# SMLC-NYSBC/TARGET-VAE

Hardware: AMD Instinct MI355X
Metric: training images/sec (fwd+bwd+Adam), P8 z=2 64x64 bs=256/GPU (higher is better)
Workload: dtype f32 (matrix products: operands as TWO fp16 parts under one power-of-two scale PER ROW of the operand (row / column of the product), 3 fp16 MFMAs per product block -- 2 where one operand is the exact 0 / 1 matrix -- fp32 accumulate: at least as accurate against fp64 as the fp32 matrix pipe (profiles/

## Files before the change

target-vae_amd/csrc/enc_tail_x6_kernels.hpp:

```cpp

#pragma once
#include <hip/hip_runtime.h>
#include "dense_x6_kernels.hpp"

namespace tvae {

constexpr int ET_C = 128;
constexpr int ET_WAVES = 8;
constexpr int ET_THREADS = 64 * ET_WAVES;
constexpr int ET_D = 4;
constexpr int ET_CHUNK = 32;
constexpr int ET_MAXH = 7;

template <int ACT>
__device__ __forceinline__ float et_act(float v, float slope) {
    if (ACT == ACT_LRELU) return v > 0.f ? v : v * slope;
    if (ACT == ACT_TANH) return tanhf(v);
    return v;
}

__device__ __forceinline__ int et_row(int i, int r, int kh) { return 32 * i + 8 * (r >> 2) + (r & 3) + 4 * kh; }

__device__ __forceinline__ void et_split2h(const float (&x)[8], float s, Cell16 (&bf)[3]) {
    const float y[8] = {x[0] * s, x[1] * s, x[2] * s, x[3] * s, x[4] * s, x[5] * s, x[6] * s, x[7] * s};
    split2hx8(y, bf[0], bf[1]);
}
template <int NP>
__device__ __forceinline__ void et_split(const float (&x)[8], Cell16 (&bf)[3]) {
    if (NP == 3) {
        split3x8(x, bf[0], bf[1], bf[2]);
    } else {
#pragma unroll
        for (int q = 0; q < 4; ++q) bf[0].w[q] = bf16_pair(x[2 * q], x[2 * q + 1]);
    }
}

template <int NP>
__device__ __forceinline__ void et_load_a(const uint4* __restrict__ Ws, int t, int i, int kh, int nl, Cell16 (&a)[3]) {
    const uint4* wp = Ws + (2 * t + kh) * ET_C + nl + 32 * i;
#pragma unroll
    for (int p = 0; p < NP; ++p) a[p].u = wp[p * 16 * ET_C];
}
template <int NP>
__device__ __forceinline__ void et_step_mfma(f32x16 (&acc)[4], const uint4* __restrict__ Ws, int t, int kh, int nl,
                                             Cell16 (&a0)[3], Cell16 (&a1)[3], const Cell16 (&bf)[3]) {
    et_load_a<NP>(Ws, t, 1, kh, nl, a1);
    mfma_np<NP>(acc[0], a0, bf);
    __builtin_amdgcn_sched_barrier(0);
    et_load_a<NP>(Ws, t, 2, kh, nl, a0);
    mfma_np<NP>(acc[1], a1, bf);
    __builtin_amdgcn_sched_barrier(0);
    et_load_a<NP>(Ws, t, 3, kh, nl, a1);
    mfma_np<NP>(acc[2], a0, bf);
    __builtin_amdgcn_sched_barrier(0);
    et_load_a<NP>(Ws, (t + 1) & 7, 0, kh, nl, a0);
    mfma_np<NP>(acc[3], a1, bf);
    __builtin_amdgcn_sched_barrier(0);
}

template <int ACT, bool FULL, bool SH = true>
__device__ __forceinline__ void et_fwd_epilogue(f32x16 (&acc)[4], const float* __restrict__ whs, float* __restrict__ H,
                                                long ldh, float* __restrict__ heads, long ldo, const float* __restrict__ bh,
                                                int nh, long n0, long N, int nl, int kh, float slope,
                                                uint4* __restrict__ bitsH) {
    float hs[8];
    unsigned hb[4] = {0u, 0u, 0u, 0u};
#pragma unroll
    for (int o = 0; o < 8; ++o) hs[o] = 0.f;
    const bool in0 = FULL || n0 + nl < N;
    const unsigned loff = (unsigned)(4 * kh * ldh + nl) * 4u;
    const float* wlane = whs + 32 * kh;
    float4 wq[2][2][2];
#pragma unroll
    for (int u = 0; u < 2; ++u) {
        wq[0][u][0] = *reinterpret_cast<const float4*>(wlane + et_row(0, u, 0) * 8);
        wq[0][u][1] = *reinterpret_cast<const float4*>(wlane + et_row(0, u, 0) * 8 + 4);
    }
#pragma unroll
    for (int it = 0; it < 32; ++it) {
        const int cur = it & 1;
        if (it + 1 < 32) {
#pragma unroll
            for (int u = 0; u < 2; ++u) {
                const int rown = et_row((2 * it + 2 + u) >> 4, (2 * it + 2 + u) & 15, 0);
                wq[cur ^ 1][u][0] = *reinterpret_cast<const float4*>(wlane + rown * 8);
                wq[cur ^ 1][u][1] = *reinterpret_cast<const float4*>(wlane + rown * 8 + 4);
            }
        }
#pragma unroll
        for (int u = 0; u < 2; ++u) {
            const int i = (2 * it + u) >> 4, r = (2 * it + u) & 15;
            const float4 w0 = wq[cur][u][0], w1 = wq[cur][u][1];
            char* hrow = reinterpret_cast<char*>(H + (long)et_row(i, r, 0) * ldh + n0);
            const float v = et_act<ACT>(acc[i][r] + w1.w, slope);
            if (ACT == ACT_LRELU) hb[i] |= v > 0.f ? (1u << (8 * (r >> 2) + (r & 3))) : 0u;
            if (SH && in0) __builtin_nontemporal_store(v, reinterpret_cast<float*>(hrow + loff));
            hs[0] = __fmaf_rn(w0.x, v, hs[0]);
            hs[1] = __fmaf_rn(w0.y, v, hs[1]);
            hs[2] = __fmaf_rn(w0.z, v, hs[2]);
            hs[3] = __fmaf_rn(w0.w, v, hs[3]);
            hs[4] = __fmaf_rn(w1.x, v, hs[4]);
            hs[5] = __fmaf_rn(w1.y, v, hs[5]);
            hs[6] = __fmaf_rn(w1.z, v, hs[6]);
        }
#pragma unroll
        for (int o = 0; o < ET_MAXH; ++o) asm volatile("" : "+v"(hs[o]));
        __builtin_amdgcn_sched_barrier(0);
    }
    if (ACT == ACT_LRELU && bitsH) {
#pragma unroll
        for (int i = 0; i < 4; ++i) {
            hb[i] <<= 4 * kh;
            hb[i] |= (unsigned)__shfl_xor((int)hb[i], 32, 64);
        }
        if (kh == 0 && in0) bitsH[n0 + nl] = make_uint4(hb[0], hb[1], hb[2], hb[3]);
    }
    float* hp = heads + n0 + nl;
#pragma unroll
    for (int q = 0; q < 4; ++q) {
        const float ve = hs[2 * q] + __shfl_xor(hs[2 * q], 32, 64);
        const float vo = (2 * q + 1 < ET_MAXH) ? hs[2 * q + 1] + __shfl_xor(hs[2 * q + 1], 32, 64) : 0.f;
        const int o = 2 * q + kh;
        if (o < nh && in0) hp[(long)o * ldo] = (kh ? vo : ve) + bh[o];
    }
}

template <int NP>
static __global__ __launch_bounds__(ET_THREADS, ET_WAVES / 4)
void enc_tail_fwd_x6_kernel(const uint4* __restrict__ W3, int Rpad, const float* __restrict__ X, long ldx,
                            const float* __restrict__ b2, const float* __restrict__ Wh, const float* __restrict__ bh, int nh,
                            float* __restrict__ H, long ldh, float* __restrict__ heads, long ldo, long N, int act,
                            float slope, uint4* __restrict__ bitsH, uint4* __restrict__ bitsA, H3Scale hs) {
    extern __shared__ __attribute__((aligned(16))) uint4 Ws[];
    __shared__ __attribute__((aligned(16))) float whs[ET_C * 8];
    __shared__ float ia_sm[NP == 2 ? ET_C : 1];
    const int tid = threadIdx.x, lane = tid & 63;
    const int wave = __builtin_amdgcn_readfirstlane(tid >> 6);
    const int nl = lane & 31, kh = lane >> 5;
    for (int i = tid; i < NP * 16 * ET_C; i += ET_THREADS) {
        const int row = i & (ET_C - 1), po = i >> 7;
        Ws[i] = W3[(long)po * Rpad + row];
    }
    if (NP == 2 && tid < ET_C) ia_sm[tid] = h3_inv(h3_scale(hs.amax_a[tid]));
    for (int i = tid; i < ET_C * 8; i += ET_THREADS) {
        const int row = i >> 3, o = i & 7;
        whs[i] = o == 7 ? (b2 ? b2[row] : 0.f) : (o < nh ? Wh[o * ET_C + row] : 0.f);
    }
    __syncthreads();

    const long nchunks = (N + ET_CHUNK - 1) / ET_CHUNK;
    const long gw = (long)blockIdx.x * (ET_THREADS / 64) + wave, gstride = (long)gridDim.x * (ET_THREADS / 64);
    if (gw >= nchunks) return;
    const long my = (nchunks - 1 - gw) / gstride + 1;

    const unsigned xlane = (unsigned)(8 * kh * ldx) * 4u;
    auto load_x = [&](long ci, int t, float (&x)[8]) {
        if (ci >= my) ci = my - 1;
        const long n0 = (gw + ci * gstride) * ET_CHUNK;
        const char* p = reinterpret_cast<const char*>(X + (long)(16 * t) * ldx + n0);
        const unsigned off = xlane + 4u * (unsigned)min((long)nl, N - 1 - n0);
#pragma unroll
        for (int j = 0; j < 8; ++j) x[j] = *reinterpret_cast<const float*>(p + (long)j * ldx * 4 + off);
    };

    f32x16 acc[4];
    float x[ET_D][8];
#pragma unroll
    for (int t = 0; t < ET_D; ++t) load_x(0, t, x[t]);
    Cell16 a0[3], a1[3];
    et_load_a<NP>(Ws, 0, 0, kh, nl, a0);
    float sx = 1.f;
    if (NP == 2) sx = h3_scale(h3_wave_max(fmaxf(hs.amax_x[lane], hs.amax_x[64 + lane])));
    const float ix = h3_inv(sx);
    for (long ci = 0; ci < my; ++ci) {
#pragma unroll
        for (int i = 0; i < 4; ++i)
#pragma unroll
            for (int r = 0; r < 16; ++r) acc[i][r] = 0.f;
        unsigned ab[4] = {0u, 0u, 0u, 0u};
#pragma unroll
        for (int t = 0; t < 8; ++t) {
            Cell16 bf[3];
            if (bitsA) {
#pragma unroll
                for (int j = 0; j < 8; ++j) ab[t >> 1] |= x[t % ET_D][j] > 0.f ? (1u << (16 * (t & 1) + j)) : 0u;
            }
            if (NP == 2) et_split2h(x[t % ET_D], sx, bf);
            else et_split<NP>(x[t % ET_D], bf);
            load_x(ci + (t + ET_D) / 8, (t + ET_D) % 8, x[t % ET_D]);
            et_step_mfma<NP>(acc, Ws, t, kh, nl, a0, a1, bf);
        }
        if (NP == 2) {
#pragma unroll
            for (int i = 0; i < 4; ++i)
#pragma unroll
                for (int r = 0; r < 16; ++r) acc[i][r] = (acc[i][r] * ia_sm[et_row(i, r, kh)]) * ix;
        }
        const long n0 = (gw + ci * gstride) * ET_CHUNK;
        if (bitsA) {
#pragma unroll
            for (int i = 0; i < 4; ++i) {
                ab[i] <<= 8 * kh;
                ab[i] |= (unsigned)__shfl_xor((int)ab[i], 32, 64);
            }
            if (kh == 0 && n0 + nl < N) bitsA[n0 + nl] = make_uint4(ab[0], ab[1], ab[2], ab[3]);
        }
#define TVAE_ET_EPI(A_)                                                                                    \
    do {                                                                                                  \
        if (!H) et_fwd_epilogue<A_, false, false>(acc, whs, H, ldh, heads, ldo, bh, nh, n0, N, nl, kh, slope, bitsH); \
        else if (n0 + ET_CHUNK <= N) et_fwd_epilogue<A_, true>(acc, whs, H, ldh, heads, ldo, bh, nh, n0, N, nl, kh, slope, bitsH); \
        else et_fwd_epilogue<A_, false>(acc, whs, H, ldh, heads, ldo, bh, nh, n0, N, nl, kh, slope, bitsH); \
    } while (0)
        if (act == ACT_LRELU) TVAE_ET_EPI(ACT_LRELU);
        else if (act == ACT_TANH) TVAE_ET_EPI(ACT_TANH);
        else TVAE_ET_EPI(ACT_NONE);
#undef TVAE_ET_EPI
    }
}

__device__ __forceinline__ float et_mask(unsigned w, int bit, float slope) { return (w >> bit) & 1u ? 1.f : slope; }

template <int NP>
static __global__ __launch_bounds__(ET_THREADS, ET_WAVES / 4)
void enc_tail_dgrad_x6_kernel(const uint4* __restrict__ W3p, int Rpad, const uint4* __restrict__ Wh3, int Rpadh,
                              const float* __restrict__ dheads, long ldd, int nh, const uint4* __restrict__ bitsH,
                              const uint4* __restrict__ bitsA, float* __restrict__ dA1, long lda, long N, float slope,
                              const float* __restrict__ amax_a) {
    constexpr int NP1 = NP == 2 ? 3 : NP;
    extern __shared__ __attribute__((aligned(16))) uint4 Ws[];
    uint4* Whs = Ws + NP * 16 * ET_C;
    const int tid = threadIdx.x, lane = tid & 63;
    const int wave = __builtin_amdgcn_readfirstlane(tid >> 6);
    const int nl = lane & 31, kh = lane >> 5;
    for (int i = tid; i < NP * 16 * ET_C; i += ET_THREADS) Ws[i] = W3p[(long)(i >> 7) * Rpad + (i & (ET_C - 1))];
    for (int i = tid; i < NP1 * 2 * ET_C; i += ET_THREADS) Whs[i] = Wh3[(long)(i >> 7) * Rpadh + (i & (ET_C - 1))];
    __shared__ float ia_sm[NP == 2 ? ET_C : 1];
    if (NP == 2 && tid < ET_C) ia_sm[tid] = h3_inv(h3_scale(amax_a[tid]));
    __syncthreads();

    const long nchunks = (N + ET_CHUNK - 1) / ET_CHUNK;
    const long gw = (long)blockIdx.x * (ET_THREADS / 64) + wave, gstride = (long)gridDim.x * (ET_THREADS / 64);
    if (gw >= nchunks) return;
    const long my = (nchunks - 1 - gw) / gstride + 1;

    float dh[8];
    uint4 wHn, wAn;
    auto load_in = [&](long ci) {
        if (ci >= my) ci = my - 1;
        const long n = min((gw + ci * gstride) * ET_CHUNK + nl, N - 1);
#pragma unroll
        for (int o = 0; o < ET_MAXH; ++o) dh[o] = o < nh ? dheads[(long)o * ldd + n] : 0.f;
        dh[7] = 0.f;
        wHn = bitsH[n];
        wAn = bitsA[n];
    };
    Cell16 dcell[3];
    unsigned wHs[4], wAs[4], wAsn[4];
    auto consume = [&]() {
        et_split<NP1>(dh, dcell);
        if (kh) {
#pragma unroll
            for (int p = 0; p < NP1; ++p) dcell[p].u = make_uint4(0u, 0u, 0u, 0u);
        }
        wHs[0] = wHn.x >> (4 * kh); wHs[1] = wHn.y >> (4 * kh); wHs[2] = wHn.z >> (4 * kh); wHs[3] = wHn.w >> (4 * kh);
        wAsn[0] = wAn.x >> (4 * kh); wAsn[1] = wAn.y >> (4 * kh); wAsn[2] = wAn.z >> (4 * kh); wAsn[3] = wAn.w >> (4 * kh);
    };
    f32x16 acc[4], G[4];
    float gs = 1.f;
    auto g_phase = [&]() {
#pragma unroll
        for (int i = 0; i < 4; ++i) {
            Cell16 wc[3];
#pragma unroll
            for (int p = 0; p < NP1; ++p) wc[p].u = Whs[(p * 2 + kh) * ET_C + 32 * i + nl];
#pragma unroll
            for (int r = 0; r < 16; ++r) G[i][r] = 0.f;
            mfma_np<NP1>(G[i], wc, dcell);
        }
        if (NP == 2) {
            float mx = 0.f;
#pragma unroll
            for (int i = 0; i < 4; ++i)
#pragma unroll
                for (int r = 0; r < 16; ++r) mx = fmaxf(mx, fabsf(G[i][r]));
            gs = h3_scale(h3_wave_max(mx));
        }
    };
    load_in(0);
    consume();
    load_in(1);
    g_phase();
    Cell16 a0[3], a1[3];
    et_load_a<NP>(Ws, 0, 0, kh, nl, a0);
    const unsigned loff = (unsigned)(4 * kh * lda + nl) * 4u;
    for (long ci = 0; ci < my; ++ci) {
#pragma unroll
        for (int i = 0; i < 4; ++i) {
            wAs[i] = wAsn[i];
#pragma unroll
            for (int r = 0; r < 16; ++r) acc[i][r] = 0.f;
        }
        const float gs_c = gs, inv_c = NP == 2 ? h3_inv(gs) : 1.f;
#pragma unroll
        for (int u = 0; u < 8; ++u) {
            float xv[8];
#pragma unroll
            for (int j = 0; j < 8; ++j) {
                const int r = 8 * (u & 1) + j;
                xv[j] = G[u >> 1][r] * et_mask(wHs[u >> 1], 8 * (r >> 2) + (r & 3), slope);
            }
            Cell16 bf[3];
            if (NP == 2) et_split2h(xv, gs_c, bf);
            else et_split<NP>(xv, bf);
            et_step_mfma<NP>(acc, Ws, u, kh, nl, a0, a1, bf);
        }
        consume();
        load_in(ci + 2);
        g_phase();
        const long n0 = (gw + ci * gstride) * ET_CHUNK;
        const bool in0 = n0 + nl < N;
#pragma unroll
        for (int i = 0; i < 4; ++i)
#pragma unroll
            for (int r = 0; r < 16; ++r) {
                char* drow = reinterpret_cast<char*>(dA1 + (long)et_row(i, r, 0) * lda + n0);
                const float v = (NP == 2 ? (acc[i][r] * ia_sm[et_row(i, r, kh)]) * inv_c : acc[i][r]) * et_mask(wAs[i], 8 * (r >> 2) + (r & 3), slope);
                if (in0) __builtin_nontemporal_store(v, reinterpret_cast<float*>(drow + loff));
            }
    }
}


constexpr int EW_NC = 32;
constexpr int EW_RAW = ET_C * EW_NC * 4;
constexpr int EW_AUX = 1024;
constexpr int EW_BITS = 1024;
constexpr int EW_STAGE = EW_RAW + EW_AUX + EW_BITS;
constexpr int EW_CELLS = 3 * 4 * ET_C * 16;
constexpr int EW_LDS = 2 * EW_STAGE + 4 * EW_CELLS;

#define TVAE_EW_DMA_X4(dst, src) \
    asm volatile("s_mov_b32 m0, %0\n\ts_nop 0\n\tglobal_load_lds_dwordx4 %1, off" ::"s"(dst), "v"(src) : "memory", "m0")

template <int NP>
static __global__ __launch_bounds__(ET_THREADS, 2) void enc_tail_wgrad_x6_kernel(
    const float* __restrict__ A1, long lda, const float* __restrict__ dheads, long ldd, int nh,
    const uint4* __restrict__ bitsH, const float* __restrict__ Wh, float* __restrict__ slabs, long N, float slope,
    const float* __restrict__ amax_a1, const float* __restrict__ amax_dh) {
    extern __shared__ __attribute__((aligned(16))) unsigned char ew_sm[];
    __shared__ float red_[NP == 2 ? 2 * ET_C : 1];
    const int tid = threadIdx.x, lane = tid & 63;
    const int wave = __builtin_amdgcn_readfirstlane(tid >> 6);
    const unsigned lds0 = (unsigned)(size_t)(__attribute__((address_space(3))) void*)ew_sm;
    uint4* cellsD = reinterpret_cast<uint4*>(ew_sm + 2 * EW_STAGE);
    uint4* cellsA = reinterpret_cast<uint4*>(ew_sm + 2 * EW_STAGE + EW_CELLS);
    const long nchunks = N / EW_NC;
    const long per = (nchunks + gridDim.x - 1) / gridDim.x;
    const long c_beg = (long)blockIdx.x * per;
    const long c_end = c_beg + per < nchunks ? c_beg + per : nchunks;
    const int row = tid & 127, oct = tid >> 7;
    float wh[ET_MAXH];
#pragma unroll
    for (int h = 0; h < ET_MAXH; ++h) wh[h] = h < nh ? Wh[(long)h * ET_C + row] : 0.f;
    float sA = 1.f, sD = 1.f;
    float* is_sm = reinterpret_cast<float*>(red_);
    if (NP == 2) {
        float rs = 0.f;
#pragma unroll
        for (int h = 0; h < ET_MAXH; ++h) rs += fabsf(wh[h]);
        sA = h3_scale(amax_a1[row]);
        sD = h3_scale(amax_dh[0] * rs);
        if (oct == 0) {
            is_sm[row] = h3_inv(sD);
            is_sm[ET_C + row] = h3_inv(sA);
        }
        __syncthreads();
    }
    const float* a_src[2];
#pragma unroll
    for (int q = 0; q < 2; ++q) {
        const int r_ = 8 * (2 * wave + q) + (lane >> 3);
        a_src[q] = A1 + (long)r_ * lda + 4 * ((lane & 7) ^ ((r_ >> 1) & 7));
    }
    const int hrow = (lane >> 3) < nh ? (lane >> 3) : 0;
    const float* h_src = dheads + (long)hrow * ldd + 4 * (lane & 7);
    auto dma_chunk = [&](long ch, int stage) {
        const long n0 = ch * EW_NC;
        const unsigned st = lds0 + (unsigned)(stage * EW_STAGE);
#pragma unroll
        for (int q = 0; q < 2; ++q) {
            const float* src = a_src[q] + n0;
            const unsigned dst = st + (unsigned)((2 * wave + q) * 1024);
            TVAE_EW_DMA_X4(dst, src);
        }
        if (wave == 1) {
            const uint4* src = bitsH + n0 + (lane & 31);
            const unsigned dst = st + (unsigned)(EW_RAW + EW_AUX);
            TVAE_EW_DMA_X4(dst, src);
        } else {
            const float* src = h_src + n0;
            const unsigned dst = st + (unsigned)EW_RAW;
            TVAE_EW_DMA_X4(dst, src);
        }
    };
    f32x16 acc[2];
#pragma unroll
    for (int j = 0; j < 2; ++j)
#pragma unroll
        for (int r = 0; r < 16; ++r) acc[j][r] = 0.f;
    const int ti = wave >> 1, tj = 2 * (wave & 1), kh = lane >> 5, li = lane & 31;
    auto build = [&](int stage, int cb) {
        const unsigned char* sb = ew_sm + stage * EW_STAGE;
        uint4* cD = cellsD + cb * (2 * EW_CELLS / 16);
        uint4* cA = cellsA + cb * (2 * EW_CELLS / 16);
        {
            const float4* rp = reinterpret_cast<const float4*>(sb + row * (EW_NC * 4));
            const int sw = (row >> 1) & 7;
            const float4 v0 = rp[(2 * oct) ^ sw], v1 = rp[(2 * oct + 1) ^ sw];
            const float x[8] = {v0.x, v0.y, v0.z, v0.w, v1.x, v1.y, v1.z, v1.w};
            Cell16 c3[3];
            if (NP == 2) et_split2h(x, sA, c3);
            else et_split<NP>(x, c3);
#pragma unroll
            for (int p = 0; p < NP; ++p) cA[(p * 4 + oct) * ET_C + row] = c3[p].u;
        }
        {
            const float* hs = reinterpret_cast<const float*>(sb + EW_RAW) + oct * 8;
            const unsigned* bw = reinterpret_cast<const unsigned*>(sb + EW_RAW + EW_AUX) + (row >> 5);
            float g[8] = {0.f, 0.f, 0.f, 0.f, 0.f, 0.f, 0.f, 0.f};
#pragma unroll
            for (int h = 0; h < ET_MAXH; ++h) {
                const float4 d0 = *reinterpret_cast<const float4*>(hs + h * EW_NC);
                const float4 d1 = *reinterpret_cast<const float4*>(hs + h * EW_NC + 4);
                g[0] = __fmaf_rn(wh[h], d0.x, g[0]); g[1] = __fmaf_rn(wh[h], d0.y, g[1]);
                g[2] = __fmaf_rn(wh[h], d0.z, g[2]); g[3] = __fmaf_rn(wh[h], d0.w, g[3]);
                g[4] = __fmaf_rn(wh[h], d1.x, g[4]); g[5] = __fmaf_rn(wh[h], d1.y, g[5]);
                g[6] = __fmaf_rn(wh[h], d1.z, g[6]); g[7] = __fmaf_rn(wh[h], d1.w, g[7]);
            }
#pragma unroll
            for (int j = 0; j < 8; ++j) {
                const unsigned w = bw[(oct * 8 + j) * 4];
                g[j] *= ((w >> (row & 31)) & 1u) ? 1.f : slope;
            }
            Cell16 c3[3];
            if (NP == 2) et_split2h(g, sD, c3);
            else et_split<NP>(g, c3);
#pragma unroll
            for (int p = 0; p < NP; ++p) cD[(p * 4 + oct) * ET_C + row] = c3[p].u;
        }
    };
    if (c_beg < c_end) {
        dma_chunk(c_beg, 0);
        asm volatile("s_waitcnt vmcnt(0)" ::: "memory");
        __syncthreads();
        dma_chunk(c_beg + 1 < c_end ? c_beg + 1 : c_beg, 1);
        build(0, 0);
    }
    for (long ch = c_beg; ch < c_end; ++ch) {
        const int cb = (int)((ch - c_beg) & 1);
        asm volatile("s_waitcnt vmcnt(0)" ::: "memory");
        __syncthreads();
        dma_chunk(ch + 2 < c_end ? ch + 2 : c_end - 1, cb);
        const uint4* cD = cellsD + cb * (2 * EW_CELLS / 16);
        const uint4* cA = cellsA + cb * (2 * EW_CELLS / 16);
#pragma unroll
        for (int ks = 0; ks < 2; ++ks) {
            Cell16 af[3], bf[2][3];
#pragma unroll
            for (int p = 0; p < NP; ++p) {
                af[p].u = cD[(p * 4 + 2 * ks + kh) * ET_C + 32 * ti + li];
                bf[0][p].u = cA[(p * 4 + 2 * ks + kh) * ET_C + 32 * tj + li];
                bf[1][p].u = cA[(p * 4 + 2 * ks + kh) * ET_C + 32 * (tj + 1) + li];
            }
            mfma_np<NP>(acc[0], af, bf[0]);
            mfma_np<NP>(acc[1], af, bf[1]);
        }
        build(cb ^ 1, cb ^ 1);
#pragma unroll
        for (int g_ = 0; g_ < 4 * NP; ++g_) {
            __builtin_amdgcn_sched_group_barrier(0x008, 1, 0);
            __builtin_amdgcn_sched_group_barrier(0x100, 3, 0);
            __builtin_amdgcn_sched_group_barrier(0x002, 14, 0);
            __builtin_amdgcn_sched_group_barrier(0x200, 1, 0);
        }
    }
    asm volatile("s_waitcnt vmcnt(0)" ::: "memory");
    float* slab = slabs + (long)blockIdx.x * ET_C * ET_C;
#pragma unroll
    for (int j = 0; j < 2; ++j)
#pragma unroll
        for (int r = 0; r < 16; ++r)
            slab[(long)et_row(ti, r, kh) * ET_C + 32 * (tj + j) + li] =
                NP == 2 ? (acc[j][r] * is_sm[et_row(ti, r, kh)]) * is_sm[ET_C + 32 * (tj + j) + li] : acc[j][r];
}

}
```

Measured before the change: 27590.

## Use 64x64 wave blocks with K-split in encoder-tail wgrad, DPP head reduction

```diff
diff --git a/target-vae_amd/csrc/enc_tail_x6_kernels.hpp b/target-vae_amd/csrc/enc_tail_x6_kernels.hpp
--- a/target-vae_amd/csrc/enc_tail_x6_kernels.hpp
+++ b/target-vae_amd/csrc/enc_tail_x6_kernels.hpp
@@ -338,6 +338,13 @@
 constexpr int EW_STAGE = EW_RAW + EW_AUX + EW_BITS;
 constexpr int EW_CELLS = 3 * 4 * ET_C * 16;
 constexpr int EW_LDS = 2 * EW_STAGE + 4 * EW_CELLS;
+#ifdef TVAE_EW_BLOCK32
+constexpr bool EW_B64 = false;
+#else
+constexpr bool EW_B64 = true;
+#endif
+constexpr int EW_PART = 4 * 64 * 64 * 4;
+static_assert(EW_PART <= 4 * EW_CELLS, "the partial sums reuse the cell sets after the loop");
 
 #define TVAE_EW_DMA_X4(dst, src) \
     asm volatile("s_mov_b32 m0, %0\n\ts_nop 0\n\tglobal_load_lds_dwordx4 %1, off" ::"s"(dst), "v"(src) : "memory", "m0")
@@ -403,12 +410,14 @@
             TVAE_EW_DMA_X4(dst, src);
         }
     };
-    f32x16 acc[2];
-#pragma unroll
-    for (int j = 0; j < 2; ++j)
+    constexpr int NACC = EW_B64 ? 4 : 2;
+    f32x16 acc[NACC];
+#pragma unroll
+    for (int j = 0; j < NACC; ++j)
 #pragma unroll
         for (int r = 0; r < 16; ++r) acc[j][r] = 0.f;
     const int ti = wave >> 1, tj = 2 * (wave & 1), kh = lane >> 5, li = lane & 31;
+    const int half = wave >> 2, bi = (wave >> 1) & 1, bj = wave & 1;
     auto build = [&](int stage, int cb) {
         const unsigned char* sb = ew_sm + stage * EW_STAGE;
         uint4* cD = cellsD + cb * (2 * EW_CELLS / 16);
@@ -428,6 +437,23 @@
             const float* hs = reinterpret_cast<const float*>(sb + EW_RAW) + oct * 8;
             const unsigned* bw = reinterpret_cast<const unsigned*>(sb + EW_RAW + EW_AUX) + (row >> 5);
             float g[8] = {0.f, 0.f, 0.f, 0.f, 0.f, 0.f, 0.f, 0.f};
+#ifndef TVAE_EW_BLOCK32
+            const int jq = (lane & 15) < 14 ? (lane & 15) : 13;
+            const float4 dq = *reinterpret_cast<const float4*>(hs + (jq >> 1) * EW_NC + 4 * (jq & 1));
+#define TVAE_EW_DPP(N_) " row_newbcast:" #N_ " row_mask:0xf bank_mask:0xf bound_ctrl:1\n\t"
+#define TVAE_EW_ROW(H_, LO_, HI_)                                                                                         \
+    asm("s_nop 1\n\t"                                                                                                     \
+        "v_fmac_f32_dpp %0, %8, %12" TVAE_EW_DPP(LO_) "v_fmac_f32_dpp %1, %9, %12" TVAE_EW_DPP(LO_)                          \
+        "v_fmac_f32_dpp %2, %10, %12" TVAE_EW_DPP(LO_) "v_fmac_f32_dpp %3, %11, %12" TVAE_EW_DPP(LO_)                        \
+        "v_fmac_f32_dpp %4, %8, %12" TVAE_EW_DPP(HI_) "v_fmac_f32_dpp %5, %9, %12" TVAE_EW_DPP(HI_)                          \
+        "v_fmac_f32_dpp %6, %10, %12" TVAE_EW_DPP(HI_) "v_fmac_f32_dpp %7, %11, %12" TVAE_EW_DPP(HI_)                        \
+        : "+v"(g[0]), "+v"(g[1]), "+v"(g[2]), "+v"(g[3]), "+v"(g[4]), "+v"(g[5]), "+v"(g[6]), "+v"(g[7])                  \
+        : "v"(dq.x), "v"(dq.y), "v"(dq.z), "v"(dq.w), "v"(wh[H_]))
+            TVAE_EW_ROW(0, 0, 1); TVAE_EW_ROW(1, 2, 3); TVAE_EW_ROW(2, 4, 5); TVAE_EW_ROW(3, 6, 7);
+            TVAE_EW_ROW(4, 8, 9); TVAE_EW_ROW(5, 10, 11); TVAE_EW_ROW(6, 12, 13);
+#undef TVAE_EW_ROW
+#undef TVAE_EW_DPP
+#else
 #pragma unroll
             for (int h = 0; h < ET_MAXH; ++h) {
                 const float4 d0 = *reinterpret_cast<const float4*>(hs + h * EW_NC);
@@ -437,6 +463,7 @@
                 g[4] = __fmaf_rn(wh[h], d1.x, g[4]); g[5] = __fmaf_rn(wh[h], d1.y, g[5]);
                 g[6] = __fmaf_rn(wh[h], d1.z, g[6]); g[7] = __fmaf_rn(wh[h], d1.w, g[7]);
             }
+#endif
 #pragma unroll
             for (int j = 0; j < 8; ++j) {
                 const unsigned w = bw[(oct * 8 + j) * 4];
@@ -463,19 +490,37 @@
         dma_chunk(ch + 2 < c_end ? ch + 2 : c_end - 1, cb);
         const uint4* cD = cellsD + cb * (2 * EW_CELLS / 16);
         const uint4* cA = cellsA + cb * (2 * EW_CELLS / 16);
-#pragma unroll
-        for (int ks = 0; ks < 2; ++ks) {
-            Cell16 af[3], bf[2][3];
-#pragma unroll
-            for (int p = 0; p < NP; ++p) {
-                af[p].u = cD[(p * 4 + 2 * ks + kh) * ET_C + 32 * ti + li];
-                bf[0][p].u = cA[(p * 4 + 2 * ks + kh) * ET_C + 32 * tj + li];
-                bf[1][p].u = cA[(p * 4 + 2 * ks + kh) * ET_C + 32 * (tj + 1) + li];
-            }
-            mfma_np<NP>(acc[0], af, bf[0]);
-            mfma_np<NP>(acc[1], af, bf[1]);
+        if (EW_B64) {
+            Cell16 af[2][3], bf[2][3];
+#pragma unroll
+            for (int p = 0; p < NP; ++p)
+#pragma unroll
+                for (int i = 0; i < 2; ++i) {
+                    af[i][p].u = cD[(p * 4 + 2 * half + kh) * ET_C + 64 * bi + 32 * i + li];
+                    bf[i][p].u = cA[(p * 4 + 2 * half + kh) * ET_C + 64 * bj + 32 * i + li];
+                }
+#pragma unroll
+            for (int pa = 0; pa < NP; ++pa)
+#pragma unroll
+                for (int pb = 0; pb < NP - pa; ++pb)
+#pragma unroll
+                    for (int t = 0; t < 4; ++t) mfma_part<NP>(acc[t], af[t >> 1][pa], bf[t & 1][pb]);
+        } else {
+#pragma unroll
+            for (int ks = 0; ks < 2; ++ks) {
+                Cell16 af[3], bf[2][3];
+#pragma unroll
+                for (int p = 0; p < NP; ++p) {
+                    af[p].u = cD[(p * 4 + 2 * ks + kh) * ET_C + 32 * ti + li];
+                    bf[0][p].u = cA[(p * 4 + 2 * ks + kh) * ET_C + 32 * tj + li];
+                    bf[1][p].u = cA[(p * 4 + 2 * ks + kh) * ET_C + 32 * (tj + 1) + li];
+                }
+                mfma_np<NP>(acc[0], af, bf[0]);
+                mfma_np<NP>(acc[1], af, bf[1]);
+            }
         }
         build(cb ^ 1, cb ^ 1);
+#ifdef TVAE_EW_BLOCK32
 #pragma unroll
         for (int g_ = 0; g_ < 4 * NP; ++g_) {
             __builtin_amdgcn_sched_group_barrier(0x008, 1, 0);
@@ -483,15 +528,38 @@
             __builtin_amdgcn_sched_group_barrier(0x002, 14, 0);
             __builtin_amdgcn_sched_group_barrier(0x200, 1, 0);
         }
+#endif
     }
     asm volatile("s_waitcnt vmcnt(0)" ::: "memory");
     float* slab = slabs + (long)blockIdx.x * ET_C * ET_C;
-#pragma unroll
-    for (int j = 0; j < 2; ++j)
-#pragma unroll
-        for (int r = 0; r < 16; ++r)
-            slab[(long)et_row(ti, r, kh) * ET_C + 32 * (tj + j) + li] =
-                NP == 2 ? (acc[j][r] * is_sm[et_row(ti, r, kh)]) * is_sm[ET_C + 32 * (tj + j) + li] : acc[j][r];
-}
-
-}
+    if (EW_B64) {
+        float* part = reinterpret_cast<float*>(ew_sm + 2 * EW_STAGE) + (wave & 3) * (64 * 64) + lane;
+        __syncthreads();
+        if (half == 1) {
+#pragma unroll
+            for (int t = 0; t < 4; ++t)
+#pragma unroll
+                for (int r = 0; r < 16; ++r) part[(16 * t + r) * 64] = acc[t][r];
+        }
+        __syncthreads();
+        if (half == 0) {
+#pragma unroll
+            for (int t = 0; t < 4; ++t)
+#pragma unroll
+                for (int r = 0; r < 16; ++r) {
+                    const int c2 = et_row(2 * bi + (t >> 1), r, kh), c = 64 * bj + 32 * (t & 1) + li;
+                    const float v = acc[t][r] + part[(16 * t + r) * 64];
+                    slab[(long)c2 * ET_C + c] = NP == 2 ? (v * is_sm[c2]) * is_sm[ET_C + c] : v;
+                }
+        }
+    } else {
+#pragma unroll
+        for (int j = 0; j < 2; ++j)
+#pragma unroll
+            for (int r = 0; r < 16; ++r)
+                slab[(long)et_row(ti, r, kh) * ET_C + 32 * (tj + j) + li] =
+                    NP == 2 ? (acc[j][r] * is_sm[et_row(ti, r, kh)]) * is_sm[ET_C + 32 * (tj + j) + li] : acc[j][r];
+    }
+}
+
+}
```

Result: no change. 27760 (median of 6 runs) (+0.6%).
